# SamShue/EKF_SLAM

Hardware: AMD Instinct MI355X
Metric: EKF update-steps/sec at N landmarks; HBM GB/s on (I−KH)P vs roofline (higher is better)
Workload: dtype f64

## Files before the change

ekf_slam_amd/csrc/gather.h:

```cpp
#pragma once

constexpr int kGatherCols = 256;
constexpr int kGatherBlock = kGatherCols + 3 * 64;

__device__ __forceinline__ double lane_bcast(double v, int src) {
    const int lo = __builtin_amdgcn_readlane(__double2loint(v), src), hi = __builtin_amdgcn_readlane(__double2hiint(v), src);
    return __hiloint2double(hi, lo);
}
__device__ __forceinline__ double lane_gather(double v, int src) {
    const int lo = __builtin_amdgcn_ds_bpermute(src << 2, __double2loint(v)), hi = __builtin_amdgcn_ds_bpermute(src << 2, __double2hiint(v));
    return __hiloint2double(hi, lo);
}
__device__ __forceinline__ double lane_xor1(double v) {
    const int lo = __builtin_amdgcn_mov_dpp(__double2loint(v), 0xB1, 0xF, 0xF, true), hi = __builtin_amdgcn_mov_dpp(__double2hiint(v), 0xB1, 0xF, 0xF, true);
    return __hiloint2double(hi, lo);
}
__device__ __forceinline__ void wave_lds_sync() { asm volatile("s_waitcnt lgkmcnt(0)" ::: "memory"); }

constexpr int kFuseMaxRows = 48;
constexpr int kFuseElems = kFuseMaxRows * kFuseMaxRows / 256;

template <typename TS>
__device__ __forceinline__ void gather_decided_other(const DevState &st, const CorrectArgs &a, const DevLoopArgs &dl, int64_t Nd,
                                                     bool append) {
// ... 94 lines not shown
        const double like = (dl.w_pos != 0.0) ? (dl.w_pos * pc + sc) : sc;
        if (like <= dl.s_thresh) { ll = like; ix = k; }
    }
    wave_argmin_sparse(ll, ix);
    if ((tid & 63) == 0) { oa_ll[tid >> 6] = ll; oa_ix[tid >> 6] = ix == INT64_MAX ? -1 : (int)ix; }
    __syncthreads();
    if (tid < 64) {
        ll = tid < kGatherCols / 64 ? oa_ll[tid] : INFINITY;
        ix = (tid < kGatherCols / 64 && oa_ix[tid] >= 0) ? (int64_t)oa_ix[tid] : INT64_MAX;
        if (ix == INT64_MAX) ll = INFINITY;
        wave_argmin_sparse(ll, ix);
        if (tid == 0) store_partial(dl.parts_out + blockIdx.x, ll, ix == INT64_MAX ? -1 : (int)ix, dl.seq_out);
    }
}

template <typename TS, bool kSharded, bool kPredict, bool kFused = false, bool kDev = false, bool kDecide = false>
__global__ __launch_bounds__(kGatherBlock) void k_gather(DevState st, CorrectArgs a, PanelView pv, PredictArgs pa,
                                                         typename DevLoopParam<kDev>::type dl) {
    static_assert(!kDev || !kFused, "the device loop never drives the small-map fused form");
    static_assert(!kDecide || (kDev && !kSharded && !kPredict), "the device-decided branch: unsharded, predict carried out before");
    __shared__ double pss[24];
    __shared__ SmallSolve sol;
    __shared__ PredictSmall ps;
    __shared__ double pose_sh[3];
    __shared__ int diag_ready;
    __shared__ int staged_cnt;
    __shared__ double2 upatch[kMaxPending * 4];
    const int tid = threadIdx.x;
    const int role = __builtin_amdgcn_readfirstlane(tid >> 6);
    const int lane = tid & 63;
    const int cur = a.cur;
    const double *__restrict__ x = cur ? st.x[1] : st.x[0];
    const double *__restrict__ strip = cur ? st.strip[1] : st.strip[0];
    const double *__restrict__ prr_cur = cur ? st.prr[1] : st.prr[0];
    double *__restrict__ x_nxt = cur ? st.x[0] : st.x[1];
    double *__restrict__ strip_nxt = cur ? st.strip[0] : st.strip[1];
    double *__restrict__ prr_nxt = cur ? st.prr[0] : st.prr[1];
    const TS *__restrict__ tiles = (const TS *)st.tiles;
    int64_t j = a.j;
    const int64_t ldm = st.ldm;
    const int npend = a.npend, pstart = a.pstart;
    if constexpr (kDev) {
        double dll;
        int dix;
        reduce_partials_wave(dl.parts_in, dl.nblk_in, dl.seq_in, lane, dll, dix);
        dix = __builtin_amdgcn_readfirstlane(dix);
        if constexpr (kDecide) {
            const int64_t Nd = dl.n_known >= 0 ? dl.n_known : *dl.dn_in;
            a.n_mm = 2 * Nd;
            const bool stopped = *(volatile int32_t *)dl.abort == dl.scan_id;
            if (stopped || !(dix >= 0 && (int64_t)dix < Nd)) {
                int code = stopped ? -3 : dix;
                if (code == -1 && *(const volatile double *)(dl.loc + 3 * (Nd - dl.loc_base) + 2) != 1.0) {
                    code = -4;
                    if (blockIdx.x == 0 && tid == kGatherCols + 64) *(volatile int32_t *)dl.abort = dl.scan_id;
                }
// ... 23 lines not shown
#define EKF_STAMP() do { } while (0)
#endif

    if (role >= 4) {
        double small_v = 0.0;
        if (role == 4) {
            const double *sp = prr_cur;
            if (lane < 9) sp = prr_cur + lane;
            else if (lane < 15) { const int t = (lane - 9) >> 1, b = (lane - 9) & 1; sp = strip + t * ldm + j + b; }
            else if (lane >= 19 && lane < 22) sp = x + (lane - 19);
            else if (lane >= 22 && lane < 24) sp = x + 3 + j + (lane - 22);
            small_v = *sp;
            if (lane == 24) { diag_ready = 0; staged_cnt = 0; }
        } else if (role == 5) {
            const int t = (lane >> 1) & 1, b = lane & 1;
            small_v = st.diag[st.dcur][3 * (j >> 1) + (t > b ? t : b) + (t > b ? b : t)];
        } else {
            small_v = x[lane < 3 ? lane : 3 + j + ((lane - 3) & 1)];
        }
        __builtin_amdgcn_sched_barrier(0);
        asm volatile("s_barrier" ::: "memory");
        EKF_STAMP();
        if (role == 4 && (lane < 15 || (lane >= 19 && lane < 24))) pss[lane] = small_v;
        if (role == 5 && lane < 4) pss[15 + lane] = small_v;
        EKF_STAMP();
        if (role == 5) {
            wave_lds_sync();
            if (lane == 0) *(volatile int *)&diag_ready = 1;
            EKF_STAMP();
        } else if (role == 6) {
            const double bx = lane_bcast(small_v, 0), by = lane_bcast(small_v, 1), bth = lane_bcast(small_v, 2),
                         blx = lane_bcast(small_v, 3), bly = lane_bcast(small_v, 4);
            if (lane == 0) {
                double pose[3] = { bx, by, bth };
                if (kPredict) {
                    const double2 sc2 = sincosd_ni(pose[2] + pa.u1);
                    const double sn2 = sc2.x, cs2 = sc2.y;
                    const double p0 = predict_pose_entry(pose, 0, pa.u0, pa.u1, sn2, cs2), p1 = predict_pose_entry(pose, 1, pa.u0, pa.u1, sn2, cs2),
                                 p2 = predict_pose_entry(pose, 2, pa.u0, pa.u1, sn2, cs2);
                    pose[0] = p0; pose[1] = p1; pose[2] = p2;
                }
                const double d0 = blx - pose[0], d1 = bly - pose[1];
                const double bearing = bearing_ni(d1, d0, pose[2]);
                const double sq = sqrt(d0 * d0 + d1 * d1);
// ... 110 lines not shown
    const int64_t c = (int64_t)blockIdx.x * kGatherCols + tid;
    const bool live = c < a.n_mm;
    static_assert(kMaxPending * 4 == 2 * kGatherCols, "two uniform operands per column lane");
    auto load_up = [&](int e0) {
        const int e = (do_patch && e0 < 4 * npend) ? e0 : 0;
        const int i = e >> 2, which = e & 3;
        const double *base = (which < 2 ? st.Kp : st.Gp) + (int64_t)ring_slot(pstart, i, st.pcap) * st.pair_stride;
        return reinterpret_cast<const double2 *>(base)[j + (which & 1)];
    };
    const double2 up0 = load_up(tid), up1 = load_up(tid + kGatherCols);
    __builtin_amdgcn_sched_barrier(0);
    asm volatile("s_barrier" ::: "memory");
    EKF_STAMP();
    double m0 = 0.0, m1 = 0.0, s0 = 0.0, s1 = 0.0, s2 = 0.0, xc = 0.0;
    const bool rowpart = c <= j, colpart = c >= j + 2;
    if (live) {
        if (kSharded) { const double2 m = pv.at(st.tm, c); m0 = m.x; m1 = m.y; }
        else if (rowpart) {
            const int64_t m = st.tm.T - 1;
            const TS *__restrict__ tp = tiles + st.tm.tile_offset(j >> st.tm.shift, c >> st.tm.shift) + ((j & m) << st.tm.shift) + (c & m);
            m0 = (double)tp[0]; m1 = (double)tp[st.tm.T];
        }
        else if (colpart) pmm_low_pair<TS>(tiles, st.tm, c, j, m0, m1);
        else pmm_low_pair<TS>(tiles, st.tm, j + 1, j, m0, m1);
        s0 = strip[c]; s1 = strip[ldm + c]; s2 = strip[2 * ldm + c];
        xc = x[3 + c];
    }
    double dgc = 0.0, dgl = 0.0;
    if (live) {
        const double *__restrict__ dg = st.diag[st.dcur] + 3 * (c >> 1);
        if (c & 1) { dgl = dg[1]; dgc = dg[2]; } else dgc = dg[0];
    }
    __builtin_amdgcn_sched_barrier(0);
    EKF_STAMP();
    upatch[tid] = up0; upatch[tid + kGatherCols] = up1;
    wave_lds_sync();
    if ((tid & 63) == 0) atomicAdd(&staged_cnt, 1);
    while (*(volatile int *)&staged_cnt < 4) { }
    wave_lds_sync();
    EKF_STAMP();

    constexpr int kPre = 32;
    const int npre = do_patch ? (npend < kPre ? npend : kPre) : 0;
    const int64_t pad_cols = st.tm.padded(a.n_mm);
// ... 12 lines not shown
        int npre_ld = npre;
        asm volatile("" : "+s"(npre_ld));
#pragma unroll
        for (int g0 = 0; g0 < kPre; g0 += 8) {
            if (g0 < npre_ld) {
#pragma unroll
                for (int t = 0; t < 8; ++t) {
                    pre[g0 + t] = *reinterpret_cast<const double2 *>(ub + (uint64_t)off * 16u + lane_bytes);
                    if (g0 + t + 1 < npre) { off += step; if (off == wrap) off = 0; }
                }
            }
        }
    }


    if (live && do_patch) {
        if (rowpart) {
#pragma unroll
            for (int g0 = 0; g0 < kPre; g0 += 8)
                if (g0 < npre) {
                    double2 ua[8], ub[8];
#pragma unroll
                    for (int t = 0; t < 8; ++t) { ua[t] = upatch[4 * (g0 + t) + 0]; ub[t] = upatch[4 * (g0 + t) + 1]; }
#pragma unroll
                    for (int t = 0; t < 8; ++t) {
                        const double v0 = rank2_apply(m0, ua[t], pre[g0 + t]), v1 = rank2_apply(m1, ub[t], pre[g0 + t]);
                        m0 = g0 + t < npre ? v0 : m0; m1 = g0 + t < npre ? v1 : m1;
                    }
                }
            const double2 *__restrict__ gp = reinterpret_cast<const double2 *>(st.Gp) + c;
            int i = npre;
            for (; i + 8 <= npend; i += 8) {
                double2 g[8];
#pragma unroll
                for (int q = 0; q < 8; ++q) g[q] = gp[(int64_t)ring_slot(pstart, i + q, st.pcap) * ps2];
#pragma unroll
                for (int q = 0; q < 8; ++q) {
                    m0 = rank2_apply(m0, upatch[4 * (i + q) + 0], g[q]);
                    m1 = rank2_apply(m1, upatch[4 * (i + q) + 1], g[q]);
                }
            }
            for (; i < npend; ++i) {
                const double2 g = gp[(int64_t)ring_slot(pstart, i, st.pcap) * ps2];
                m0 = rank2_apply(m0, upatch[4 * i + 0], g);
                m1 = rank2_apply(m1, upatch[4 * i + 1], g);
            }
        } else if (colpart) {
#pragma unroll
            for (int g0 = 0; g0 < kPre; g0 += 8)
                if (g0 < npre) {
                    double2 ua[8], ub[8];
#pragma unroll
                    for (int t = 0; t < 8; ++t) { ua[t] = upatch[4 * (g0 + t) + 2]; ub[t] = upatch[4 * (g0 + t) + 3]; }
#pragma unroll
                    for (int t = 0; t < 8; ++t) {
                        const double v0 = rank2_apply(m0, pre[g0 + t], ua[t]), v1 = rank2_apply(m1, pre[g0 + t], ub[t]);
                        m0 = g0 + t < npre ? v0 : m0; m1 = g0 + t < npre ? v1 : m1;
                    }
                }
            const double2 *__restrict__ kp = reinterpret_cast<const double2 *>(st.Kp) + c;
            int i = npre;
            for (; i + 8 <= npend; i += 8) {
                double2 k[8];
#pragma unroll
                for (int q = 0; q < 8; ++q) k[q] = kp[(int64_t)ring_slot(pstart, i + q, st.pcap) * ps2];
#pragma unroll
                for (int q = 0; q < 8; ++q) {
                    m0 = rank2_apply(m0, k[q], upatch[4 * (i + q) + 2]);
                    m1 = rank2_apply(m1, k[q], upatch[4 * (i + q) + 3]);
                }
            }
            for (; i < npend; ++i) {
                const double2 k = kp[(int64_t)ring_slot(pstart, i, st.pcap) * ps2];
                m0 = rank2_apply(m0, k, upatch[4 * i + 2]);
                m1 = rank2_apply(m1, k, upatch[4 * i + 3]);
            }
        } else {
            for (int i = 0; i < npend; ++i) {
                m0 = rank2_apply(m0, upatch[4 * i + 1], upatch[4 * i + 2]);
                m1 = rank2_apply(m1, upatch[4 * i + 1], upatch[4 * i + 3]);
            }
        }
    }
    {
        const double dgl_p = lane_xor1(dgl);
        if (c == j) { m0 = dgc; m1 = dgl_p; }
        else if (c == j + 1) { m0 = dgl; m1 = dgc; }
    }
    EKF_STAMP();
    __syncthreads();
    EKF_STAMP();

    const int64_t pad_end = st.tm.padded(a.n_mm);
    const int64_t out_off = (int64_t)ring_slot(pstart, npend, st.pcap) * st.pair_stride;
    double2 *__restrict__ Gout = reinterpret_cast<double2 *>(st.Gp + out_off);
    double2 *__restrict__ Kout = reinterpret_cast<double2 *>(st.Kp + out_off);
    double g[2] = { 0.0, 0.0 }, k0 = 0.0, k1 = 0.0;
    double xn = 0.0, t0 = 0.0, t1 = 0.0, t2 = 0.0;
    if (live) {
        if (kPredict) predict_strip(s0, s1, s2, ps.fa, ps.fb);
        for (int r = 0; r < 2; ++r)
            g[r] = sol.Hs[r][0] * s0 + sol.Hs[r][1] * s1 + sol.Hs[r][2] * s2 + sol.Hs[r][3] * m0 + sol.Hs[r][4] * m1;
        k0 = g[0] * sol.Phi[0] + g[1] * sol.Phi[2];
        k1 = g[0] * sol.Phi[1] + g[1] * sol.Phi[3];
        if (!kFused) {
            Gout[c] = make_double2(g[0], g[1]);
            Kout[c] = make_double2(k0, k1);
            if (st.Gp32) {
                st.Gp32[out_off + c] = (float)g[0]; st.Gp32[out_off + ldm + c] = (float)g[1];
                st.Kp32[out_off + c] = -(float)k0; st.Kp32[out_off + ldm + c] = -(float)k1;
            }
        }
        xn = xc + (k0 * sol.nu[0] + k1 * sol.nu[1]);
        t0 = s0 - (sol.Kr[0][0] * g[0] + sol.Kr[0][1] * g[1]);
        t1 = s1 - (sol.Kr[1][0] * g[0] + sol.Kr[1][1] * g[1]);
        t2 = s2 - (sol.Kr[2][0] * g[0] + sol.Kr[2][1] * g[1]);
        x_nxt[3 + c] = xn;
        double *__restrict__ sn = strip_nxt;
        sn[c] = t0;
        sn[ldm + c] = t1;
        sn[2 * ldm + c] = t2;
    } else if (c < pad_end && !kFused) {
        Gout[c] = make_double2(0.0, 0.0);
        Kout[c] = make_double2(0.0, 0.0);
        if (st.Gp32) {
            st.Gp32[out_off + c] = 0.0f; st.Gp32[out_off + ldm + c] = 0.0f;
            st.Kp32[out_off + c] = -0.0f; st.Kp32[out_off + ldm + c] = -0.0f;
        }
    }
    double ndc, ndl;
    {
        const double2 kn = make_double2(k0, k1), gn = make_double2(g[0], g[1]);
        const double2 gl = make_double2(lane_xor1(gn.x), lane_xor1(gn.y));
        ndc = rank2_apply(dgc, kn, gn);
        ndl = rank2_apply(dgl, kn, gl);
        if (live) {
// ... 86 lines not shown
```

ekf_slam_amd/csrc/host/assoc.h:

```cpp
#pragma once
namespace {
struct PartView { double ll; int32_t index; int32_t seq; };
inline PartView read_part(const volatile AssocHostPartial *e) {
    const volatile uint64_t *w = reinterpret_cast<const volatile uint64_t *>(e);
    const uint64_t lo = w[0], hi = w[1];
    PartView v;
    memcpy(&v.ll, &lo, 8);
    v.index = (int32_t)(uint32_t)(hi & 0xffffffffu);
    v.seq = (int32_t)((uint32_t)(hi >> 32) - assoc_part_mix((uint32_t)(lo & 0xffffffffu), (uint32_t)(lo >> 32), (uint32_t)v.index));
    return v;
}

int32_t verify_loop(ekf_handle *h, bool block) {
    if (h->lrec_tail == h->lrec_head) return EKF_OK;
    if (block) {
        const volatile AssocHostPartial *newest = h->h_lrec + (h->lrec_head - 1) % ekf_handle::kLoopRing;
        const int32_t want = h->lspec.back().seq;
        bool landed = false;
        for (int spin = 0; spin < 200000 && !landed; ++spin) { landed = read_part(newest).seq == want; if (!landed) __builtin_ia32_pause(); }
        if (!landed) HIPCHK(h, hipStreamSynchronize(h->stream));
        __atomic_thread_fence(__ATOMIC_ACQUIRE);
    }
    size_t done = 0;
    int32_t rc = EKF_OK;
// ... 67 lines not shown
    return EKF_OK;
}

int32_t collect_decision(ekf_handle *h, AssocHostPartial *set, int32_t nblk, int32_t seq, int64_t N, bool may_poll, int32_t *is_new,
                         int64_t *idx) {
    if (!(may_poll && h->assoc_poll && wait_parts(set, nblk, seq))) {
        HIPCHK(h, hipStreamSynchronize(h->stream));
        __atomic_thread_fence(__ATOMIC_ACQUIRE);
    }
    return reduce_parts(h, set, nblk, seq, N, is_new, idx);
}

int32_t launch_assoc(ekf_handle *h, const double z[3], const double R[4], AssocHostPartial *host_set_dev, int32_t seq,
                     bool exchange = false, bool want_costs = false, bool fold_predict = false) {
    REQUIRE(h, h->N >= 1, EKF_ERR_STATE, "associate: the state holds no landmark (Correspondence.m:29)");
    if (!fold_predict) {
        const int32_t rcp = materialize_predict(h);
        if (rcp) return rcp;
    }
    AssocArgs a;
    a.z0 = z[0]; a.z1 = z[1]; a.z2 = z[2];
    colmajor2(R, a.R00, a.R01, a.R10, a.R11);
    a.s_cost = h->cfg.s_cost; a.s_thresh = h->cfg.s_thresh; a.w_pos = h->cfg.w_pos;
    a.N = h->N; a.cur = h->cur; a.npend = h->npend; a.pstart = h->pstart;
    a.own_only = exchange ? 1 : 0;
    TimedLaunch tl(h, EKF_KERNEL_ASSOCIATE);
    HIPCHK(h, launch_associate(h->st, a, exchange ? (want_costs ? h->send + 4 : nullptr) : h->d_pos_cost, h->d_sig_cost,
                               h->d_partial, h->d_ticket, h->d_decision, exchange ? nullptr : host_set_dev, seq,
                               exchange ? h->send : nullptr, h->storage, h->stream, (fold_predict && h->have_pp) ? &h->pp : nullptr));
    if (fold_predict && h->have_pp) { h->have_pp = false; h->cur ^= 1; }
    return EKF_OK;
}
// ... 183 lines not shown
```

ekf_slam_amd/csrc/host/edits.h:

```cpp
#pragma once
namespace {
int32_t edit_unsharded(ekf_handle *h, const std::string &who, const char *why) {
    if (h->cfg.world == 1) return EKF_OK;
    return fail(h, EKF_ERR_INVALID_ARG, (who + "not built for sharded handles (world > 1): " + why).c_str());
}

int32_t edit_settled(ekf_handle *h, const std::string &who) {
    if (h->pending) return fail(h, EKF_ERR_STATE, (who + "a sharded correction is between begin and finish").c_str());
    const int32_t rc = use_device(h);
    return rc ? rc : verify_loop(h,  true);
}

int32_t edit_flushed(ekf_handle *h) { TRY(materialize_predict(h)); return flush_pending(h); }

const char *parse_R(const double R[4], double &r00, double &r01, double &r10, double &r11) {
    r00 = r01 = r10 = r11 = 0.0;
    if (R) colmajor2(R, r00, r01, r10, r11);
    if (!(std::isfinite(r00) && std::isfinite(r01) && std::isfinite(r10) && std::isfinite(r11))) return "R is not finite";
    if (!(r01 == r10 && r00 >= 0.0 && r11 >= 0.0 && r00 * r11 - r01 * r10 >= 0.0)) return "R must be symmetric with non-negative diagonal and determinant";
    return nullptr;
}

int32_t removal_alloc(ekf_handle *h) {
    const int64_t nmap = h->st.ldm / 2;
    const bool first_removal = !h->tilebuf[1] || !h->d_cmap || !h->d_s_tmp;
    if (!h->tilebuf[1]) {
        char *tiles2 = nullptr;
        HIPCHK(h, dalloc(h, &tiles2, (size_t)h->work_cap * h->T * h->T * elt_size(h)));
// ... 285 lines not shown
```

ekf_slam_amd/csrc/host/handle.h:

```cpp
#pragma once
#include "../../../include/ekfslam.h"
#include <hip/hip_runtime.h>
#include <dlfcn.h>
#include <cstdio>
#include <cstdlib>
#include <algorithm>
#include <cmath>
#include <cstring>
#include <new>
#include <string>
#include <vector>

#include "../device_math.h"
#include "../flush32_pipe.h"
#include "../kernels.h"
#include "../layout.h"

struct KernelTimer {
    bool enabled = false;
    std::vector<hipEvent_t> ev;
    size_t used = 0;
};

struct ekf_handle {
    ekf_config cfg;
    int64_t N = 0;
    int64_t cap = 0;
    int32_t T = 64;
    int32_t storage = 0;
    int32_t cur = 0;
    DevState st;
    hipStream_t own_stream = nullptr, stream = nullptr;
    double *h_small = nullptr;
    double *d_digest = nullptr;
    bool have_pp = false;
    PredictArgs pp;
    std::vector<double> s_host;
    mutable std::vector<std::pair<double, int64_t>> s_sorted, s_tail;
    mutable bool s_sorted_ok = false;
    static constexpr size_t kSortedTail = 2048;
    hipEvent_t throttle_ev[2] = { nullptr, nullptr };
    bool throttle_set[2] = { false, false };
    int throttle_k = 0, since_mark = 0;
    int32_t batch = 1;
    int32_t npend = 0;
    int32_t pstart = 0;
    bool async_flush = false;
    void *tilebuf[2] = { nullptr, nullptr };
    int32_t base = 0;
    int32_t nfrozen = 0;
    bool inflight = false;
// ... 198 lines not shown
```

ekf_slam_amd/csrc/host/lifecycle.h:

```cpp
#pragma once
namespace {
int32_t create_state(ekf_handle *h) {
    const int64_t ldm = h->st.ldm;
    for (int b = 0; b < 2; ++b) {
        HIPCHK(h, dalloc(h, &h->st.x[b], (size_t)(3 + ldm)));
        HIPCHK(h, dalloc(h, &h->st.prr[b], 16));
        HIPCHK(h, dalloc(h, &h->st.strip[b], (size_t)(3 * ldm)));
        HIPCHK(h, dalloc(h, &h->st.diag[b], (size_t)(3 * h->cap)));
    }
    h->st.dcur = 0;
    HIPCHK(h, dalloc(h, &h->st.s, (size_t)h->cap));
    HIPCHK(h, dalloc(h, &h->st.small, 32));
    HIPCHK(h, dalloc(h, &h->d_digest, kDigestDoubles));
    HIPCHK(h, dalloc(h, &h->d_csmall, 16));
    HIPCHK(h, halloc(h, &h->h_small, 32 * sizeof(double), hipHostMallocDefault));
    const double prr0[9] = { 0.1, 0, 0, 0, 0.1, 0, 0, 0, 0.1 };
    HIPCHK(h, hipMemcpy(h->st.prr[0], prr0, sizeof prr0, hipMemcpyHostToDevice));
    h->cur = 0;
    h->N = 0;
    return EKF_OK;
}
}

extern "C" {
// ... 40 lines not shown
    h->work_cap = h->st.tm.slots_for_rows(nt_cap);

    TRY(create_state(h));
    TRY(create_passes(h, prop));
    TRY(create_worklists(h));
    TRY(create_assoc(h));
    TRY(create_exchange(h));
    TRY(create_decided(h));
    HIPCHK(h, hipDeviceSynchronize());
    return EKF_OK;
}

int32_t ekf_destroy(ekf_handle *h) {
    if (!h) return EKF_OK;
    hipSetDevice(h->cfg.device);
    if (h->stream) hipStreamSynchronize(h->stream);
    if (h->comm && g_rccl.CommDestroy) g_rccl.CommDestroy(h->comm);
    for (hipStream_t s : { h->flush_stream, h->xchg_stream }) if (s) { hipStreamSynchronize(s); hipStreamDestroy(s); }
    for (hipEvent_t e : h->events) hipEventDestroy(e);
    for (auto &t : h->timers) for (hipEvent_t e : t.ev) hipEventDestroy(e);
    for (void *p : h->allocs) hipFree(p);
    for (void *p : h->pinned) hipHostFree(p);
    if (h->own_stream) hipStreamDestroy(h->own_stream);
    delete h;
    return EKF_OK;
}

int32_t ekf_kernel_timing_enable(ekf_handle *h, int32_t which, int32_t on) {
    if (!h || which < 0 || which >= EKF_KERNEL_COUNT) return fail(h, EKF_ERR_INVALID_ARG, "kernel_timing_enable: bad kernel id");
    TRY(use_device(h));
// ... 35 lines not shown
```

ekf_slam_amd/csrc/host/measure.h:

```cpp
#pragma once
namespace {
struct Scan { const double *obs; int64_t m; const double *u, *lm_index, *lm_loc; int64_t L; };
struct Winners { bool have; int set; int32_t seq, nblk; };

void ride_next(ekf_handle *h, const Scan &sc, int64_t row, int set_out, int64_t n_mm_after, DevLoopArgs &dl, Winners &nxt) {
    dl.parts_out = h->d_lparts + (int64_t)set_out * h->lparts_stride;
    dl.seq_out = next_assoc_seq(h);
    dl.z0 = sc.obs[row]; dl.z1 = sc.obs[sc.m + row]; dl.z2 = sc.obs[2 * sc.m + row];
    dl.R00 = dl.z0 * h->cfg.Rc[0]; dl.R01 = 0.0; dl.R10 = 0.0; dl.R11 = dl.z1 * h->cfg.Rc[1];
    dl.s_cost = h->cfg.s_cost; dl.s_thresh = h->cfg.s_thresh; dl.w_pos = h->cfg.w_pos;
    nxt.have = true; nxt.set = set_out; nxt.seq = dl.seq_out; nxt.nblk = (int32_t)gather_workgroups(h->st, n_mm_after);
}

int32_t measure_row_empty(ekf_handle *h, const Scan &sc, const double R[4]) {
    double loc[2];
    const int32_t rc = lookup_loc(h, sc.lm_index, sc.lm_loc, sc.L, true, 0.0, loc);
    return rc ? rc : do_append(h, sc.u, R, loc, 1.0);
}

int32_t measure_decided_rows(ekf_handle *h, const Scan &sc, int64_t first, int tab_set, int64_t kbase) {
    const double *obs = sc.obs, *u = sc.u;
    const int64_t m = sc.m;
    Winners nxt = { false, 0, 0, 0 };
    for (int64_t ii = first; ii < m; ++ii) {
        const double z[3] = { obs[ii], obs[m + ii], obs[2 * m + ii] };
        const double R[4] = { z[0] * h->cfg.Rc[0], 0.0, 0.0, z[1] * h->cfg.Rc[1] };
        if (!nxt.have) {
            nxt.set = h->loop_set ^ 1; nxt.seq = next_assoc_seq(h);
            AssocArgs a = {};
            a.z0 = z[0]; a.z1 = z[1]; a.z2 = z[2];
            colmajor2(R, a.R00, a.R01, a.R10, a.R11);
            a.s_cost = h->cfg.s_cost; a.s_thresh = h->cfg.s_thresh; a.w_pos = h->cfg.w_pos;
            a.N = n_hi(h); a.cur = h->cur; a.npend = h->npend; a.pstart = h->pstart; a.own_only = 0;
            a.dN = unsettled(h) > 0 ? h->d_nring + h->nrow % ekf_handle::kNRing : nullptr;
            nxt.nblk = assoc_blocks(a.N);
            TIMED(h, EKF_KERNEL_ASSOCIATE, launch_associate_devn(h->st, a, h->d_lparts + (int64_t)nxt.set * h->lparts_stride, nxt.seq, h->storage,
                  h->stream, h->have_pp ? &h->pp : nullptr));
            if (h->have_pp) { h->have_pp = false; h->cur ^= 1; }
// ... 208 lines not shown
```

ekf_slam_amd/csrc/host/passes.h:

```cpp
#pragma once
namespace {
int32_t refresh_work(ekf_handle *h) {
    const int64_t nt = ekf_tiles_for(2 * n_hi(h), h->T);
    if (nt == h->ws[h->ws_cur].rows) return EKF_OK;
    const int32_t to = h->ws_pass == h->ws_cur ? h->ws_cur ^ 1 : h->ws_cur;
    ekf_handle::WorkSet &ws = h->ws[to];
    const size_t b_work = (size_t)h->work_cap * sizeof(int2), b_xcd = 8 * b_work, b_segs = (size_t)h->segs_cap * sizeof(int4);
    if (!h->wl_stage) h->wl_stage_bytes = b_work + b_xcd + b_segs;
    int32_t rc = stage_alloc(h, &h->wl_stage, h->wl_stage_bytes, &h->ev_wl);
    if (!rc) rc = stage_wait(h, h->ev_wl, h->wl_busy);
    if (rc) return rc;
    int2 *w = reinterpret_cast<int2 *>(h->wl_stage);
    int2 *flat = reinterpret_cast<int2 *>(h->wl_stage + b_work);
    int4 *segs = reinterpret_cast<int4 *>(h->wl_stage + b_work + b_xcd);
    size_t nw = 0;
    REQUIRE(h, h->st.tm.slots_for_rows(nt) <= h->work_cap, EKF_ERR_STATE, "work list overflow");
    for (int64_t I = 0; I < nt; ++I)
        for (int64_t J = 0; J <= I; ++J)
            if (h->st.tm.mine(I, J)) w[nw++] = make_int2((int)I, (int)J);
    if (nw) HIPCHK(h, hipMemcpyAsync(ws.work, w, nw * sizeof(int2), hipMemcpyHostToDevice, h->stream));
    ws.nwork = (int64_t)nw;
    ws.rows = nt;

    static const int S = std::max(1, ekf_tune_int("EKF_SUPERTILE", 8));
// ... 64 lines not shown
    job.grid_cap = h->grid_cap; job.arith = h->cfg.pass_arith;
    job.aux = pass_aux(h, ws, ax);
    return job;
}

int32_t create_worklists(ekf_handle *h) {
    for (auto &ws : h->ws) {
        if (h->cfg.pass_arith != EKF_ARITH_F64) HIPCHK(h, dalloc(h, &ws.segs, (size_t)h->segs_cap));
        HIPCHK(h, dalloc(h, &ws.work, (size_t)h->work_cap));
        HIPCHK(h, dalloc(h, &ws.xcd, (size_t)h->work_cap * 8));
    }
    return EKF_OK;
}

int32_t retire_inflight(ekf_handle *h) {
    if (!h->inflight) return EKF_OK;
    if (h->appended_inflight) {
        if (!h->ev_rows) HIPCHK(h, new_event(h, &h->ev_rows));
        HIPCHK(h, hipEventRecord(h->ev_rows, h->stream));
        HIPCHK(h, hipStreamWaitEvent(h->flush_stream, h->ev_rows, 0));
        if (decided_mode(h)) {
            const int64_t *hi = unsettled(h) > 0 ? h->d_nring + h->nrow % ekf_handle::kNRing : nullptr;
            HIPCHK(h, launch_copy_rows_dev(h->st.tm, h->tilebuf[h->base], h->tilebuf[h->base ^ 1], 2 * h->inflight_N, 2 * n_hi(h), h->inflight_dn,
                                           hi, h->storage, h->flush_stream));
        } else
            HIPCHK(h, launch_copy_rows(h->st.tm, h->tilebuf[h->base], h->tilebuf[h->base ^ 1], 2 * h->inflight_N, 2 * h->N, h->storage, h->flush_stream));
        HIPCHK(h, hipEventRecord(h->ev_flushed, h->flush_stream));
        h->appended_inflight = false;
    }
    HIPCHK(h, hipStreamWaitEvent(h->stream, h->ev_flushed, 0));
// ... 6 lines not shown
    h->inflight = false;
    tiles_changed(h);
    return EKF_OK;
}

void next_pass_direction(ekf_handle *h) {
    const int force = h->cfg.pass_direction == 1 ? 0 : h->cfg.pass_direction == 2 ? 1 : -1;
    constexpr int64_t kCacheBytes = 256ll << 20;
    const int64_t nt = ekf_tiles_for(2 * n_hi(h), h->T);
    const int64_t store = nt * (nt + 1) / 2 / std::max(1, h->cfg.world) * (int64_t)h->T * h->T * (h->storage == EKF_STORE_F64 ? 8 : 4);
    const bool alternate = force >= 0 ? force != 0 : store > kCacheBytes;
    h->st.tm.reverse = alternate ? (h->st.tm.reverse ^ 1) : 0;
}

int32_t flush_pending(ekf_handle *h, bool batch_done = false) {
    TRY(retire_inflight(h));
    if (h->npend == 0) return EKF_OK;
    TRY(refresh_work(h));
    next_pass_direction(h);
    bool extracted = false;
    const int64_t hint = h->hint_idx;
    bool pn = false, pn_side = false;
    if (batch_done && !h->pn_idx.empty()) {
        if (h->sharded && !h->pending && h->pn_N == h->N && (h->comm || h->xhook)) {
            const int32_t m = (int32_t)h->pn_idx.size();
            const int64_t slab = slab_for(h, n_mm(h));
            TIMED(h, EKF_KERNEL_ROWPANEL, launch_rowpanel_next(h->st, h->pn_idx.data(), m, n_mm(h), h->pstart, h->npend, h->send, slab, h->storage,
                  h->stream));
            tiles_changed(h);
            h->pf_idx = h->pn_idx; h->pf_m = m; h->pf_slab = slab; h->pf_N = h->N;
// ... 35 lines not shown
        PassJob job = pass_job(h, ws, h->st.tiles, ax);
        job.nx = nx.j >= 0 ? &nx : nullptr;
        HIPCHK(h, launch_downdate(h->st, job, h->storage, h->stream, h->dd_kernel, &extracted));
        h->dd_pairs = h->npend;
    }
    h->npend = 0;
    h->pstart = 0;
    h->pf_valid = pn;
    if (pn_side) HIPCHK(h, hipStreamWaitEvent(h->stream, h->ev_pn_done, 0));
    h->nx_valid = extracted && !pn;
    if (extracted) { h->nx_idx = hint; h->nx_N = h->N; }
    return EKF_OK;
}

int32_t batch_complete(ekf_handle *h) {
    if (!h->async_flush) return flush_pending(h,  true);
    HIPCHK(h, hipEventRecord(h->ev_pairs, h->stream));
    h->ws_unordered = false;
    TRY(retire_inflight(h));
    TRY(refresh_work(h));
    HIPCHK(h, hipStreamWaitEvent(h->flush_stream, h->ev_pairs, 0));
    if (h->ws_unordered) HIPCHK(h, hipStreamWaitEvent(h->flush_stream, h->ev_wl, 0));
    {
        TimedLaunch tl(h, EKF_KERNEL_DOWNDATE, h->flush_stream);
        next_pass_direction(h);
        const ekf_handle::WorkSet &ws = h->ws[h->ws_cur];
        PassAux ax;
        HIPCHK(h, launch_downdate(h->st, pass_job(h, ws, h->tilebuf[h->base ^ 1], ax), h->storage, h->flush_stream, h->dd_kernel));
        h->dd_pairs = h->npend;
    }
// ... 74 lines not shown
```

ekf_slam_amd/csrc/host/steps.h:

```cpp
#pragma once
namespace {
int32_t verify_loop(ekf_handle *h, bool block);
void note_append(ekf_handle *h, double signature);

int32_t materialize_predict(ekf_handle *h) {
    if (!h->have_pp) return EKF_OK;
    h->have_pp = false;
    PredictArgs a = h->pp;
    a.n_mm = 2 * n_hi(h); a.cur = h->cur;
    TIMED(h, EKF_KERNEL_PREDICT, launch_predict(h->st, a, h->storage, h->stream));
    h->cur ^= 1;
    return EKF_OK;
}

int32_t do_predict(ekf_handle *h, const double u[2]) {
    TRY(materialize_predict(h));
    h->pp.u0 = u[0]; h->pp.u1 = u[1]; h->pp.C = h->cfg.C; h->pp.n_mm = 0; h->pp.cur = 0;
    h->have_pp = true;
    static const bool lazy = ekf_tune_int("EKF_LAZY_PREDICT", 1) != 0;
    return lazy ? EKF_OK : materialize_predict(h);
}

int32_t enter(ekf_handle *h) {
    HIPCHK(h, hipSetDevice(h->cfg.device));
    const int32_t rc = verify_loop(h,  true);
    return rc ? rc : materialize_predict(h);
}

int32_t enter_flushed(ekf_handle *h) { TRY(enter(h)); return flush_pending(h); }

int32_t do_append(ekf_handle *h, const double u[2], const double R[4], const double pos[2], double signature,
                  const DevLoopArgs *dl = nullptr) {
    REQUIRE(h, h->N < h->cap, EKF_ERR_CAPACITY, "append: capacity_landmarks exhausted");
    if (h->inflight) h->appended_inflight = true;
    AppendArgs a;
    a.u0 = u[0]; a.u1 = u[1];
    colmajor2(R, a.R00, a.R01, a.R10, a.R11);
    a.pos0 = pos[0]; a.pos1 = pos[1]; a.signature = signature; a.N = h->N; a.cur = h->cur;
    {
        PredictArgs pa = h->pp;
        pa.n_mm = n_mm(h); pa.cur = h->cur;
        const PredictArgs *fuse = h->have_pp ? &pa : nullptr;
        TIMED(h, EKF_KERNEL_APPEND, launch_append(h->st, a, h->storage, h->stream, dl, fuse));
        if (fuse) { h->have_pp = false; h->cur ^= 1; }
    }
    note_append(h, signature);
    return EKF_OK;
}

void note_append(ekf_handle *h, double signature) {
    if ((int64_t)h->s_host.size() > h->N) { h->s_host.resize((size_t)h->N); h->s_sorted_ok = false; }
    h->s_host.push_back(signature);
    if (h->s_sorted_ok && signature == signature)
        h->s_tail.emplace_back(signature, h->N);
    h->N += 1;
    map_grew(h);
}

constexpr int kThrottle = 48;

// ... 86 lines not shown
    REQUIRE(h, idx >= 0 && idx < h->N, EKF_ERR_INDEX, "correct: landmark index outside the state");
    if (h->sharded) {
        const int q = prefetch_slot(h, idx);
        if (q >= 0 && slab_for(h, n_mm(h)) == h->pf_slab) {
            REQUIRE(h, !h->pending, EKF_ERR_STATE, "correct: an exchange is pending");
            CorrectArgs a;
            fill_correct_args(h, a, z, R, idx);
            const int32_t rc = gather_sharded(h, a, h->pf_store, (int64_t)h->pf_m * h->pf_slab, (int64_t)q * h->pf_slab,  false);
            return rc ? rc : finish_step(h);
        }
        int32_t rc = correct_begin(h, z, R, idx);
        if (!rc) rc = run_exchange(h);
        return rc ? rc : correct_finish(h);
    }
    TRY(refresh_work(h));
    CorrectArgs a;
    fill_correct_args(h, a, z, R, idx);
    static const bool fuse_small = ekf_tune_int("EKF_FUSE_SMALL", 1) != 0;
    const bool fused = fuse_small && h->batch == 1 && !h->async_flush && h->npend == 0 && a.n_mm <= gather_fuse_max_rows() &&
                       ekf_tiles_for(a.n_mm, h->T) * h->T <= 256;
    const PredictArgs *fuse = h->have_pp ? &h->pp : nullptr;
    TIMED(h, EKF_KERNEL_GATHER, launch_gather(h->st, a, fuse, h->storage, h->stream, fused));
    h->have_pp = false;
    if (fused) {
        h->cur ^= 1;
        h->st.dcur ^= 1;
        snprintf(h->dd_kernel, sizeof h->dd_kernel, "k_gather<%s,fused downdate>", h->storage == EKF_STORE_F64 ? "double" : "float");
        h->dd_pairs = 1;
        return throttle_step(h);
    }
    return finish_step(h);
}

int32_t do_correct_dev(ekf_handle *h, const double z[2], const double R[4], int64_t idx, const DevLoopArgs &dl) {
    REQUIRE(h, idx >= 0 && idx < h->N, EKF_ERR_INDEX, "correct: landmark index outside the state");
    TRY(refresh_work(h));
    CorrectArgs a;
    fill_correct_args(h, a, z, R, idx);
    if (h->sharded) {
        REQUIRE(h, !h->pending, EKF_ERR_STATE, "correct: an exchange is pending");
        h->slab = slab_for(h, a.n_mm);
        TIMED(h, EKF_KERNEL_ROWPANEL, launch_rowpanel_dev(h->st, a.j, a.n_mm, h->pstart, h->npend, corr_send(h, h->slab), h->storage, h->stream, dl));
        exchange_changed(h);
        h->x_count = h->slab;
        TRY(exchange_bracket(h, 1));
        TRY(gather_sharded(h, a, h->recv, h->slab, 0,  true, &dl));
        return finish_step(h);
    }
    const PredictArgs *fuse = h->have_pp ? &h->pp : nullptr;
    TIMED(h, EKF_KERNEL_GATHER, launch_gather_devloop(h->st, a, fuse, dl, h->storage, h->stream));
// ... 60 lines not shown
```

ekf_slam_amd/csrc/kernels.h:

```cpp
#pragma once
#include <hip/hip_runtime.h>
#include <stdint.h>

#include "layout.h"

#ifdef EKF_TUNING
#include <stdlib.h>
inline int ekf_tune_int(const char *name, int dflt) { const char *v = getenv(name); return v ? atoi(v) : dflt; }
#else
constexpr int ekf_tune_int(const char *, int dflt) { return dflt; }
#endif

struct DevState {
    double *x[2];
    double *prr[2];
    double *strip[2];
    void   *tiles;
    double *s;
    double *Gp;
    double *Kp;
    float  *Gp32;
    float  *Kp32;
    int64_t pair_stride;
    int32_t pcap;
// ... 42 lines not shown
hipError_t launch_append(const DevState &st, const AppendArgs &a, int storage, hipStream_t s, const DevLoopArgs *dl = nullptr,
                         const PredictArgs *fused_predict = nullptr);

struct CorrectArgs {
    double z0, z1;
    double R00, R01, R10, R11;
    int64_t j;
    int64_t n_mm;
    int32_t cur;
    int32_t npend;
    int32_t pstart;
};
hipError_t launch_gather(const DevState &st, const CorrectArgs &a, const PredictArgs *fused_predict, int storage,
                         hipStream_t s, bool fuse_downdate);
int gather_fuse_max_rows();
hipError_t launch_gather_devloop(const DevState &st, const CorrectArgs &a, const PredictArgs *fused_predict, const DevLoopArgs &dl,
                                 int storage, hipStream_t s);
int64_t gather_workgroups(const DevState &st, int64_t n_mm);
hipError_t launch_gather_decided(const DevState &st, const CorrectArgs &a, const DevLoopArgs &dl, int storage, hipStream_t s);

hipError_t launch_rowpanel(const DevState &st, int64_t j, int64_t n_mm, int pstart, int npend, double *send, int storage,
                           hipStream_t s);
hipError_t launch_rowpanel_dev(const DevState &st, int64_t j, int64_t n_mm, int pstart, int npend, double *send, int storage,
                               hipStream_t s, const DevLoopArgs &dl);
struct RowList { int32_t m; int32_t j[64]; };
hipError_t launch_rowpanel_base(const DevState &st, const int64_t *idx, int m, int64_t n_mm, double *send, int64_t slab,
                                int storage, hipStream_t s);
hipError_t launch_rowpanel_next(const DevState &st, const int64_t *idx, int m, int64_t n_mm, int pstart, int npend, double *send,
                                int64_t slab, int storage, hipStream_t s);
hipError_t launch_gather_sharded(const DevState &st, const CorrectArgs &a, const PredictArgs *fused_predict, const double *recv,
// ... 106 lines not shown
```

ekf_slam_amd/csrc/launch/steps.h:

```cpp
#pragma once

hipError_t launch_predict(const DevState &st, const PredictArgs &a, int, hipStream_t s) {
    static const int force = ekf_tune_int("EKF_PREDICT_MFMA", -1);
    const bool mfma = force >= 0 ? force != 0 : a.n_mm >= 2048;
    if (mfma) {
        const int64_t nslices = (a.n_mm + 15) / 16;
        int64_t grid = cdiv(nslices > 0 ? nslices : 1, 4);
        if (grid > 1024) grid = 1024;
        hipLaunchKernelGGL(k_predict_mfma, dim3((unsigned)grid), dim3(kBlock), 0, s, st, a);
        return hipGetLastError();
    }
    const int64_t grid = cdiv(a.n_mm > 0 ? a.n_mm : 1, kBlock);
    hipLaunchKernelGGL(k_predict, dim3((unsigned)grid), dim3(kBlock), 0, s, st, a);
    return hipGetLastError();
}

hipError_t launch_append(const DevState &st, const AppendArgs &a, int storage, hipStream_t s, const DevLoopArgs *dlp,
                         const PredictArgs *fused_predict) {
    const int64_t n_mm = 2 * a.N;
    const int64_t grid = cdiv(n_mm > 0 ? n_mm : 1, kBlock);
    const DevLoopArgs dl = dlp ? *dlp : DevLoopArgs{};
    const PredictArgs pa = predict_or_none(fused_predict);
    return with_storage(storage, [&](auto ts) { with_bool(fused_predict != nullptr, [&](auto pred) {
        hipLaunchKernelGGL((k_append<decltype(ts), decltype(pred)::value>), dim3((unsigned)grid), dim3(kBlock), 0, s, st, a, dl, pa);
// ... 18 lines not shown
        auto launch = [&](auto pred) {
            hipLaunchKernelGGL((k_gather<decltype(ts), kSharded, decltype(pred)::value, kFused, kDev, kDecide>), dim3((unsigned)grid),
                               dim3(kGatherBlock), 0, s, st, a, pv, pa, dla);
        };
        if constexpr (kDecide) launch(std::false_type{});
        else with_bool(fused_predict != nullptr, launch);
    });
}
}

hipError_t launch_gather(const DevState &st, const CorrectArgs &a, const PredictArgs *fused_predict, int storage,
                         hipStream_t s, bool fuse_downdate) {
    if (!fuse_downdate) return gather_form<false, false, false, false>(st, a, fused_predict, PanelView{}, nullptr, storage, s);
    if (a.n_mm > kFuseMaxRows || gather_workgroups(st, a.n_mm) != 1) return hipErrorInvalidValue;
    return gather_form<false, true, false, false>(st, a, fused_predict, PanelView{}, nullptr, storage, s);
}

hipError_t launch_gather_devloop(const DevState &st, const CorrectArgs &a, const PredictArgs *fused_predict, const DevLoopArgs &dl,
                                 int storage, hipStream_t s) {
    return gather_form<false, false, true, false>(st, a, fused_predict, PanelView{}, &dl, storage, s);
}

hipError_t launch_gather_decided(const DevState &st, const CorrectArgs &a, const DevLoopArgs &dl, int storage, hipStream_t s) {
    if (!dl.dn_out || !dl.loc || !dl.abort || (dl.n_known < 0 && !dl.dn_in)) return hipErrorInvalidValue;
    return gather_form<false, false, true, true>(st, a, nullptr, PanelView{}, &dl, storage, s);
}

hipError_t launch_gather_sharded(const DevState &st, const CorrectArgs &a, const PredictArgs *fused_predict, const double *recv,
                                 int64_t rank_stride, int64_t offset, bool patched, int storage, hipStream_t s, const DevLoopArgs *dl) {
    const PanelView pv = { recv, rank_stride, offset,  a.j >> st.tm.shift, patched ? 1 : 0 };
// ... 90 lines not shown
```

Baseline: 1925.

## Defer landmark append and fuse it into the next correction gather kernel

Appending a landmark is now recorded lazily on the host instead of launched at once. When the next correction targets an existing landmark, the append work runs inside the gather kernel: the new rows' strip, covariance blocks and cross-covariance entries are built in-kernel for the two appended columns and written to the tiles. This removes a separate append kernel launch and a pass over the state per new landmark. The cost is extra template complexity and many flush points that must issue the pending append, with correctness risk around ordering.

```diff
diff --git a/ekf_slam_amd/csrc/gather.h b/ekf_slam_amd/csrc/gather.h
--- a/ekf_slam_amd/csrc/gather.h
+++ b/ekf_slam_amd/csrc/gather.h
@@ -132,10 +132,14 @@
     }
 }
 
-template <typename TS, bool kSharded, bool kPredict, bool kFused = false, bool kDev = false, bool kDecide = false>
+template <bool kDev, bool kAppend> struct GatherExtra { using type = typename DevLoopParam<kDev>::type; };
+template <> struct GatherExtra<false, true> { using type = AppendArgs; };
+
+template <typename TS, bool kSharded, bool kPredict, bool kFused = false, bool kDev = false, bool kDecide = false, bool kAppend = false>
 __global__ __launch_bounds__(kGatherBlock) void k_gather(DevState st, CorrectArgs a, PanelView pv, PredictArgs pa,
-                                                         typename DevLoopParam<kDev>::type dl) {
+                                                         typename GatherExtra<kDev, kAppend>::type dl) {
     static_assert(!kDev || !kFused, "the device loop never drives the small-map fused form");
+    static_assert(!kAppend || (!kSharded && !kFused && !kDev), "the append rides in the plain unsharded form only");
     static_assert(!kDecide || (kDev && !kSharded && !kPredict), "the device-decided branch: unsharded, predict carried out before");
     __shared__ double pss[24];
     __shared__ SmallSolve sol;
@@ -158,6 +162,13 @@
     int64_t j = a.j;
     const int64_t ldm = st.ldm;
     const int npend = a.npend, pstart = a.pstart;
+    double *ajx = nullptr;
+    int64_t n_old = a.n_mm;
+    if constexpr (kAppend) {
+        __shared__ double ajx_sh[2];
+        ajx = ajx_sh;
+        n_old = 2 * dl.N;
+    }
     if constexpr (kDev) {
         double dll;
         int dix;
@@ -211,7 +222,11 @@
             if (lane == 24) { diag_ready = 0; staged_cnt = 0; }
         } else if (role == 5) {
             const int t = (lane >> 1) & 1, b = lane & 1;
-            small_v = st.diag[st.dcur][3 * (j >> 1) + (t > b ? t : b) + (t > b ? b : t)];
+            if constexpr (!kAppend) small_v = st.diag[st.dcur][3 * (j >> 1) + (t > b ? t : b) + (t > b ? b : t)];
+            else {
+                const double *sp = st.diag[st.dcur] + (3 * (j >> 1) + (t > b ? t : b) + (t > b ? b : t));
+                small_v = *(lane < 4 ? sp : x + 2);
+            }
         } else {
             small_v = x[lane < 3 ? lane : 3 + j + ((lane - 3) & 1)];
         }
@@ -225,6 +240,13 @@
             wave_lds_sync();
             if (lane == 0) *(volatile int *)&diag_ready = 1;
             EKF_STAMP();
+            if constexpr (kAppend) {
+                double hd[3] = { 0.0, 0.0, lane_bcast(small_v, 4) };
+                if (kPredict) hd[2] = predict_pose_entry(hd, 2, pa.u0, pa.u1, 0.0, 0.0);
+                double jxr[2][3];
+                append_jxr(dl.u0, hd[2], jxr);
+                if (lane == 0) { ajx[0] = jxr[0][2]; ajx[1] = jxr[1][2]; }
+            }
         } else if (role == 6) {
             const double bx = lane_bcast(small_v, 0), by = lane_bcast(small_v, 1), bth = lane_bcast(small_v, 2),
                          blx = lane_bcast(small_v, 3), bly = lane_bcast(small_v, 4);
@@ -365,7 +387,8 @@
     EKF_STAMP();
     double m0 = 0.0, m1 = 0.0, s0 = 0.0, s1 = 0.0, s2 = 0.0, xc = 0.0;
     const bool rowpart = c <= j, colpart = c >= j + 2;
-    if (live) {
+    const bool stored = kAppend ? c < n_old : live;
+    if (stored) {
         if (kSharded) { const double2 m = pv.at(st.tm, c); m0 = m.x; m1 = m.y; }
         else if (rowpart) {
             const int64_t m = st.tm.T - 1;
@@ -378,7 +401,7 @@
         xc = x[3 + c];
     }
     double dgc = 0.0, dgl = 0.0;
-    if (live) {
+    if (stored) {
         const double *__restrict__ dg = st.diag[st.dcur] + 3 * (c >> 1);
         if (c & 1) { dgl = dg[1]; dgc = dg[2]; } else dgc = dg[0];
     }
@@ -421,7 +444,38 @@
     }
 
 
-    if (live && do_patch) {
+    auto patch_colpart = [&](double &m0, double &m1) {
+#pragma unroll
+        for (int g0 = 0; g0 < kPre; g0 += 8)
+            if (g0 < npre) {
+                double2 ua[8], ub[8];
+#pragma unroll
+                for (int t = 0; t < 8; ++t) { ua[t] = upatch[4 * (g0 + t) + 2]; ub[t] = upatch[4 * (g0 + t) + 3]; }
+#pragma unroll
+                for (int t = 0; t < 8; ++t) {
+                    const double v0 = rank2_apply(m0, pre[g0 + t], ua[t]), v1 = rank2_apply(m1, pre[g0 + t], ub[t]);
+                    m0 = g0 + t < npre ? v0 : m0; m1 = g0 + t < npre ? v1 : m1;
+                }
+            }
+        const double2 *__restrict__ kp = reinterpret_cast<const double2 *>(st.Kp) + c;
+        int i = npre;
+        for (; i + 8 <= npend; i += 8) {
+            double2 k[8];
+#pragma unroll
+            for (int q = 0; q < 8; ++q) k[q] = kp[(int64_t)ring_slot(pstart, i + q, st.pcap) * ps2];
+#pragma unroll
+            for (int q = 0; q < 8; ++q) {
+                m0 = rank2_apply(m0, k[q], upatch[4 * (i + q) + 2]);
+                m1 = rank2_apply(m1, k[q], upatch[4 * (i + q) + 3]);
+            }
+        }
+        for (; i < npend; ++i) {
+            const double2 k = kp[(int64_t)ring_slot(pstart, i, st.pcap) * ps2];
+            m0 = rank2_apply(m0, k, upatch[4 * i + 2]);
+            m1 = rank2_apply(m1, k, upatch[4 * i + 3]);
+        }
+    };
+    if (stored && do_patch) {
         if (rowpart) {
 #pragma unroll
             for (int g0 = 0; g0 < kPre; g0 += 8)
@@ -452,37 +506,8 @@
                 m0 = rank2_apply(m0, upatch[4 * i + 0], g);
                 m1 = rank2_apply(m1, upatch[4 * i + 1], g);
             }
-        } else if (colpart) {
-#pragma unroll
-            for (int g0 = 0; g0 < kPre; g0 += 8)
-                if (g0 < npre) {
-                    double2 ua[8], ub[8];
-#pragma unroll
-                    for (int t = 0; t < 8; ++t) { ua[t] = upatch[4 * (g0 + t) + 2]; ub[t] = upatch[4 * (g0 + t) + 3]; }
-#pragma unroll
-                    for (int t = 0; t < 8; ++t) {
-                        const double v0 = rank2_apply(m0, pre[g0 + t], ua[t]), v1 = rank2_apply(m1, pre[g0 + t], ub[t]);
-                        m0 = g0 + t < npre ? v0 : m0; m1 = g0 + t < npre ? v1 : m1;
-                    }
-                }
-            const double2 *__restrict__ kp = reinterpret_cast<const double2 *>(st.Kp) + c;
-            int i = npre;
-            for (; i + 8 <= npend; i += 8) {
-                double2 k[8];
-#pragma unroll
-                for (int q = 0; q < 8; ++q) k[q] = kp[(int64_t)ring_slot(pstart, i + q, st.pcap) * ps2];
-#pragma unroll
-                for (int q = 0; q < 8; ++q) {
-                    m0 = rank2_apply(m0, k[q], upatch[4 * (i + q) + 2]);
-                    m1 = rank2_apply(m1, k[q], upatch[4 * (i + q) + 3]);
-                }
-            }
-            for (; i < npend; ++i) {
-                const double2 k = kp[(int64_t)ring_slot(pstart, i, st.pcap) * ps2];
-                m0 = rank2_apply(m0, k, upatch[4 * i + 2]);
-                m1 = rank2_apply(m1, k, upatch[4 * i + 3]);
-            }
-        } else {
+        } else if (colpart) patch_colpart(m0, m1);
+        else {
             for (int i = 0; i < npend; ++i) {
                 m0 = rank2_apply(m0, upatch[4 * i + 1], upatch[4 * i + 2]);
                 m1 = rank2_apply(m1, upatch[4 * i + 1], upatch[4 * i + 3]);
@@ -505,7 +530,32 @@
     double g[2] = { 0.0, 0.0 }, k0 = 0.0, k1 = 0.0;
     double xn = 0.0, t0 = 0.0, t1 = 0.0, t2 = 0.0;
     if (live) {
-        if (kPredict) predict_strip(s0, s1, s2, ps.fa, ps.fb);
+        if (kPredict && stored) predict_strip(s0, s1, s2, ps.fa, ps.fb);
+        if constexpr (kAppend) {
+            if (!stored) {
+                const int b = (int)(c - n_old);
+                const double jxr[2][3] = { { 1, 0, ajx[0] }, { 0, 1, ajx[1] } };
+                double prr_p[9], cblk[3], iblk[3][2];
+#pragma unroll
+                for (int i = 0; i < 9; ++i) prr_p[i] = pss[i];
+                append_blocks(jxr, prr_p, dl.u0, dl.u1, dl.R00, dl.R01, dl.R10, dl.R11, cblk, iblk);
+                m0 = (double)(TS)append_row_entry(jxr, b, pss[9], pss[11], pss[13]);
+                m1 = (double)(TS)append_row_entry(jxr, b, pss[10], pss[12], pss[14]);
+                patch_colpart(m0, m1);
+                s0 = iblk[0][b]; s1 = iblk[1][b]; s2 = iblk[2][b];
+                xc = b ? dl.pos1 : dl.pos0;
+                TS *__restrict__ tw = (TS *)st.tiles;
+                if (b == 0) {
+                    dgc = cblk[0];
+                    pmm_low_store<TS>(tw, st.tm, n_old, n_old, cblk[0]);
+                    st.s[dl.N] = dl.signature;
+                } else {
+                    dgl = cblk[1]; dgc = cblk[2];
+                    pmm_low_store<TS>(tw, st.tm, n_old + 1, n_old, cblk[1]);
+                    pmm_low_store<TS>(tw, st.tm, n_old + 1, n_old + 1, cblk[2]);
+                }
+            }
+        }
         for (int r = 0; r < 2; ++r)
             g[r] = sol.Hs[r][0] * s0 + sol.Hs[r][1] * s1 + sol.Hs[r][2] * s2 + sol.Hs[r][3] * m0 + sol.Hs[r][4] * m1;
         k0 = g[0] * sol.Phi[0] + g[1] * sol.Phi[2];
@@ -527,6 +577,14 @@
         sn[c] = t0;
         sn[ldm + c] = t1;
         sn[2 * ldm + c] = t2;
+        if constexpr (kAppend) {
+            if (stored) {
+                const double jxr[2][3] = { { 1, 0, ajx[0] }, { 0, 1, ajx[1] } };
+                TS *__restrict__ tw = (TS *)st.tiles;
+#pragma unroll
+                for (int i = 0; i < 2; ++i) pmm_low_store<TS>(tw, st.tm, n_old + i, c, append_row_entry(jxr, i, s0, s1, s2));
+            }
+        }
     } else if (c < pad_end && !kFused) {
         Gout[c] = make_double2(0.0, 0.0);
         Kout[c] = make_double2(0.0, 0.0);
diff --git a/ekf_slam_amd/csrc/host/assoc.h b/ekf_slam_amd/csrc/host/assoc.h
--- a/ekf_slam_amd/csrc/host/assoc.h
+++ b/ekf_slam_amd/csrc/host/assoc.h
@@ -105,8 +105,8 @@
 int32_t launch_assoc(ekf_handle *h, const double z[3], const double R[4], AssocHostPartial *host_set_dev, int32_t seq,
                      bool exchange = false, bool want_costs = false, bool fold_predict = false) {
     REQUIRE(h, h->N >= 1, EKF_ERR_STATE, "associate: the state holds no landmark (Correspondence.m:29)");
-    if (!fold_predict) {
-        const int32_t rcp = materialize_predict(h);
+    if (!fold_predict || h->have_ap) {
+        const int32_t rcp = issue_recorded(h);
         if (rcp) return rcp;
     }
     AssocArgs a;
diff --git a/ekf_slam_amd/csrc/host/edits.h b/ekf_slam_amd/csrc/host/edits.h
--- a/ekf_slam_amd/csrc/host/edits.h
+++ b/ekf_slam_amd/csrc/host/edits.h
@@ -11,7 +11,7 @@
     return rc ? rc : verify_loop(h,  true);
 }
 
-int32_t edit_flushed(ekf_handle *h) { TRY(materialize_predict(h)); return flush_pending(h); }
+int32_t edit_flushed(ekf_handle *h) { TRY(issue_recorded(h)); return flush_pending(h); }
 
 const char *parse_R(const double R[4], double &r00, double &r01, double &r10, double &r11) {
     r00 = r01 = r10 = r11 = 0.0;
diff --git a/ekf_slam_amd/csrc/host/handle.h b/ekf_slam_amd/csrc/host/handle.h
--- a/ekf_slam_amd/csrc/host/handle.h
+++ b/ekf_slam_amd/csrc/host/handle.h
@@ -35,6 +35,8 @@
     double *d_digest = nullptr;
     bool have_pp = false;
     PredictArgs pp;
+    bool have_ap = false;
+    AppendArgs ap;
     std::vector<double> s_host;
     mutable std::vector<std::pair<double, int64_t>> s_sorted, s_tail;
     mutable bool s_sorted_ok = false;
diff --git a/ekf_slam_amd/csrc/host/lifecycle.h b/ekf_slam_amd/csrc/host/lifecycle.h
--- a/ekf_slam_amd/csrc/host/lifecycle.h
+++ b/ekf_slam_amd/csrc/host/lifecycle.h
@@ -78,6 +78,7 @@
 int32_t ekf_destroy(ekf_handle *h) {
     if (!h) return EKF_OK;
     hipSetDevice(h->cfg.device);
+    issue_recorded(h);
     if (h->stream) hipStreamSynchronize(h->stream);
     if (h->comm && g_rccl.CommDestroy) g_rccl.CommDestroy(h->comm);
     for (hipStream_t s : { h->flush_stream, h->xchg_stream }) if (s) { hipStreamSynchronize(s); hipStreamDestroy(s); }
diff --git a/ekf_slam_amd/csrc/host/measure.h b/ekf_slam_amd/csrc/host/measure.h
--- a/ekf_slam_amd/csrc/host/measure.h
+++ b/ekf_slam_amd/csrc/host/measure.h
@@ -22,6 +22,7 @@
     const double *obs = sc.obs, *u = sc.u;
     const int64_t m = sc.m;
     Winners nxt = { false, 0, 0, 0 };
+    TRY(issue_append(h));
     for (int64_t ii = first; ii < m; ++ii) {
         const double z[3] = { obs[ii], obs[m + ii], obs[2 * m + ii] };
         const double R[4] = { z[0] * h->cfg.Rc[0], 0.0, 0.0, z[1] * h->cfg.Rc[1] };
diff --git a/ekf_slam_amd/csrc/host/passes.h b/ekf_slam_amd/csrc/host/passes.h
--- a/ekf_slam_amd/csrc/host/passes.h
+++ b/ekf_slam_amd/csrc/host/passes.h
@@ -1,5 +1,7 @@
 #pragma once
 namespace {
+int32_t issue_append(ekf_handle *h);
+
 int32_t refresh_work(ekf_handle *h) {
     const int64_t nt = ekf_tiles_for(2 * n_hi(h), h->T);
     if (nt == h->ws[h->ws_cur].rows) return EKF_OK;
@@ -102,6 +104,7 @@
 }
 
 int32_t retire_inflight(ekf_handle *h) {
+    TRY(issue_append(h));
     if (!h->inflight) return EKF_OK;
     if (h->appended_inflight) {
         if (!h->ev_rows) HIPCHK(h, new_event(h, &h->ev_rows));
@@ -138,6 +141,7 @@
 }
 
 int32_t flush_pending(ekf_handle *h, bool batch_done = false) {
+    TRY(issue_append(h));
     TRY(retire_inflight(h));
     if (h->npend == 0) return EKF_OK;
     TRY(refresh_work(h));
@@ -203,6 +207,7 @@
 }
 
 int32_t batch_complete(ekf_handle *h) {
+    TRY(issue_append(h));
     if (!h->async_flush) return flush_pending(h,  true);
     HIPCHK(h, hipEventRecord(h->ev_pairs, h->stream));
     h->ws_unordered = false;
diff --git a/ekf_slam_amd/csrc/host/steps.h b/ekf_slam_amd/csrc/host/steps.h
--- a/ekf_slam_amd/csrc/host/steps.h
+++ b/ekf_slam_amd/csrc/host/steps.h
@@ -3,7 +3,7 @@
 int32_t verify_loop(ekf_handle *h, bool block);
 void note_append(ekf_handle *h, double signature);
 
-int32_t materialize_predict(ekf_handle *h) {
+int32_t issue_predict(ekf_handle *h) {
     if (!h->have_pp) return EKF_OK;
     h->have_pp = false;
     PredictArgs a = h->pp;
@@ -13,18 +13,37 @@
     return EKF_OK;
 }
 
+int32_t launch_append_now(ekf_handle *h, AppendArgs a, const DevLoopArgs *dl) {
+    if (h->inflight) h->appended_inflight = true;
+    a.cur = h->cur;
+    PredictArgs pa = h->pp;
+    pa.n_mm = 2 * a.N; pa.cur = h->cur;
+    const PredictArgs *fuse = h->have_pp ? &pa : nullptr;
+    TIMED(h, EKF_KERNEL_APPEND, launch_append(h->st, a, h->storage, h->stream, dl, fuse));
+    if (fuse) { h->have_pp = false; h->cur ^= 1; }
+    return EKF_OK;
+}
+
+int32_t issue_append(ekf_handle *h) {
+    if (!h->have_ap) return EKF_OK;
+    h->have_ap = false;
+    return launch_append_now(h, h->ap, nullptr);
+}
+
+int32_t issue_recorded(ekf_handle *h) { return h->have_ap ? issue_append(h) : issue_predict(h); }
+
 int32_t do_predict(ekf_handle *h, const double u[2]) {
-    TRY(materialize_predict(h));
+    TRY(issue_recorded(h));
     h->pp.u0 = u[0]; h->pp.u1 = u[1]; h->pp.C = h->cfg.C; h->pp.n_mm = 0; h->pp.cur = 0;
     h->have_pp = true;
     static const bool lazy = ekf_tune_int("EKF_LAZY_PREDICT", 1) != 0;
-    return lazy ? EKF_OK : materialize_predict(h);
+    return lazy ? EKF_OK : issue_predict(h);
 }
 
 int32_t enter(ekf_handle *h) {
     HIPCHK(h, hipSetDevice(h->cfg.device));
     const int32_t rc = verify_loop(h,  true);
-    return rc ? rc : materialize_predict(h);
+    return rc ? rc : issue_recorded(h);
 }
 
 int32_t enter_flushed(ekf_handle *h) { TRY(enter(h)); return flush_pending(h); }
@@ -32,18 +51,14 @@
 int32_t do_append(ekf_handle *h, const double u[2], const double R[4], const double pos[2], double signature,
                   const DevLoopArgs *dl = nullptr) {
     REQUIRE(h, h->N < h->cap, EKF_ERR_CAPACITY, "append: capacity_landmarks exhausted");
-    if (h->inflight) h->appended_inflight = true;
+    TRY(issue_append(h));
     AppendArgs a;
     a.u0 = u[0]; a.u1 = u[1];
     colmajor2(R, a.R00, a.R01, a.R10, a.R11);
     a.pos0 = pos[0]; a.pos1 = pos[1]; a.signature = signature; a.N = h->N; a.cur = h->cur;
-    {
-        PredictArgs pa = h->pp;
-        pa.n_mm = n_mm(h); pa.cur = h->cur;
-        const PredictArgs *fuse = h->have_pp ? &pa : nullptr;
-        TIMED(h, EKF_KERNEL_APPEND, launch_append(h->st, a, h->storage, h->stream, dl, fuse));
-        if (fuse) { h->have_pp = false; h->cur ^= 1; }
-    }
+    static const bool lazy = ekf_tune_int("EKF_LAZY_APPEND", 1) != 0;
+    if (lazy && !h->sharded && dl == nullptr) { h->ap = a; h->have_ap = true; }
+    else TRY(launch_append_now(h, a, dl));
     note_append(h, signature);
     return EKF_OK;
 }
@@ -160,12 +175,20 @@
         return rc ? rc : correct_finish(h);
     }
     TRY(refresh_work(h));
+    static const bool fuse_small = ekf_tune_int("EKF_FUSE_SMALL", 1) != 0;
+    const bool fused = fuse_small && h->batch == 1 && !h->async_flush && h->npend == 0 && n_mm(h) <= gather_fuse_max_rows() &&
+                       ekf_tiles_for(n_mm(h), h->T) * h->T <= 256;
+    if (h->have_ap && (fused || idx == h->ap.N)) TRY(issue_append(h));
     CorrectArgs a;
     fill_correct_args(h, a, z, R, idx);
-    static const bool fuse_small = ekf_tune_int("EKF_FUSE_SMALL", 1) != 0;
-    const bool fused = fuse_small && h->batch == 1 && !h->async_flush && h->npend == 0 && a.n_mm <= gather_fuse_max_rows() &&
-                       ekf_tiles_for(a.n_mm, h->T) * h->T <= 256;
     const PredictArgs *fuse = h->have_pp ? &h->pp : nullptr;
+    if (h->have_ap) {
+        if (h->inflight) h->appended_inflight = true;
+        TIMED(h, EKF_KERNEL_GATHER, launch_gather_append(h->st, a, h->ap, fuse, h->storage, h->stream));
+        h->have_ap = false;
+        h->have_pp = false;
+        return finish_step(h);
+    }
     TIMED(h, EKF_KERNEL_GATHER, launch_gather(h->st, a, fuse, h->storage, h->stream, fused));
     h->have_pp = false;
     if (fused) {
@@ -180,6 +203,7 @@
 
 int32_t do_correct_dev(ekf_handle *h, const double z[2], const double R[4], int64_t idx, const DevLoopArgs &dl) {
     REQUIRE(h, idx >= 0 && idx < h->N, EKF_ERR_INDEX, "correct: landmark index outside the state");
+    TRY(issue_append(h));
     TRY(refresh_work(h));
     CorrectArgs a;
     fill_correct_args(h, a, z, R, idx);
diff --git a/ekf_slam_amd/csrc/kernels.h b/ekf_slam_amd/csrc/kernels.h
--- a/ekf_slam_amd/csrc/kernels.h
+++ b/ekf_slam_amd/csrc/kernels.h
@@ -80,6 +80,8 @@
 hipError_t launch_gather(const DevState &st, const CorrectArgs &a, const PredictArgs *fused_predict, int storage,
                          hipStream_t s, bool fuse_downdate);
 int gather_fuse_max_rows();
+hipError_t launch_gather_append(const DevState &st, const CorrectArgs &a, const AppendArgs &ap, const PredictArgs *fused_predict, int storage,
+                                hipStream_t s);
 hipError_t launch_gather_devloop(const DevState &st, const CorrectArgs &a, const PredictArgs *fused_predict, const DevLoopArgs &dl,
                                  int storage, hipStream_t s);
 int64_t gather_workgroups(const DevState &st, int64_t n_mm);
diff --git a/ekf_slam_amd/csrc/launch/steps.h b/ekf_slam_amd/csrc/launch/steps.h
--- a/ekf_slam_amd/csrc/launch/steps.h
+++ b/ekf_slam_amd/csrc/launch/steps.h
@@ -56,6 +56,17 @@
     if (!fuse_downdate) return gather_form<false, false, false, false>(st, a, fused_predict, PanelView{}, nullptr, storage, s);
     if (a.n_mm > kFuseMaxRows || gather_workgroups(st, a.n_mm) != 1) return hipErrorInvalidValue;
     return gather_form<false, true, false, false>(st, a, fused_predict, PanelView{}, nullptr, storage, s);
+}
+
+hipError_t launch_gather_append(const DevState &st, const CorrectArgs &a, const AppendArgs &ap, const PredictArgs *fused_predict, int storage,
+                                hipStream_t s) {
+    if (st.tm.world != 1 || a.n_mm != 2 * ap.N + 2 || a.j < 0 || a.j >= 2 * ap.N) return hipErrorInvalidValue;
+    const int64_t grid = gather_workgroups(st, a.n_mm);
+    const PredictArgs pa = predict_or_none(fused_predict);
+    return with_storage(storage, [&](auto ts) { with_bool(fused_predict != nullptr, [&](auto pred) {
+        hipLaunchKernelGGL((k_gather<decltype(ts), false, decltype(pred)::value, false, false, false, true>), dim3((unsigned)grid),
+                           dim3(kGatherBlock), 0, s, st, a, PanelView{}, pa, ap);
+    }); });
 }
 
 hipError_t launch_gather_devloop(const DevState &st, const CorrectArgs &a, const PredictArgs *fused_predict, const DevLoopArgs &dl,
```

New measurement: 1925. No clear change (-0.0%).
